# Richard-coder/uvio

Hardware: AMD Instinct MI355X
Metric: VIO frames/sec (track+propagate+update) at clones x feats (higher is better)
Workload: dtype f64

## Files before the change

include/uvio_hp.h:

```cpp
#ifndef UVIO_HP_H
#define UVIO_HP_H

#include <stddef.h>
#include <stdint.h>

#ifdef __cplusplus
extern "C" {
#endif

#define UVIO_HP_OK 0
#define UVIO_HP_E_ARG (-1)
#define UVIO_HP_E_STATE (-2)
#define UVIO_HP_E_DEVICE (-3)
#define UVIO_HP_E_NUMERIC (-4)
#define UVIO_HP_E_CONFIG (-5)
#define UVIO_HP_E_ORDER (-6)
#define UVIO_HP_E_CAPACITY (-7)
#define UVIO_HP_E_INTERNAL (-8)

#define UVIO_HP_MAX_CAMS 4
#define UVIO_HP_MAX_ANCHORS 16
#define UVIO_HP_AUX_MAX_DIM 8


// ... 208 lines not shown
int uvio_hp_aux_init_p(double *P, int N, int ld, int dim, const int *H_index, int n, const double *H_x, int ldhx,
                       const double *H_auxinv, const double *res_unused_or_null, const double *R, int ldr);
int uvio_hp_aux_walk_p(double *P, int N, int ld, int ntab, const int *ids, const int *dims, const double *sigma2,
                       double dt);
int uvio_hp_debug_position_update_p(double *P, int N, int ld, int imu_id, const double *q, const double *p, int aux_id,
                                    const double *s, int r, const double *C, const double *z, const double *R, int ldr,
                                    double chi2_thr, double *dx, double *chi2, int *applied);
int uvio_hp_chi2_95(int dof, double *thr);
int uvio_hp_msckf_compressed_update(double *P, int N, const int *H_index, int n, const double *H, int m,
                                    const double *res, double sigma2, double *dx_out);
int uvio_hp_compress(const double *A, int m, int n, double *R_out);
int uvio_hp_undistort(int model, const double cam[8], int n, const float *uv, float *uvn, uint8_t *ambiguous);
int uvio_hp_debug_grid_order(const uint8_t *resp, const int *off, int ncell, int kmax, int depth, int *arrangement,
                             int *top);
int uvio_hp_debug_clahe(const uint8_t *img, int w, int h, int stride, uint8_t *out);
typedef struct {
  uint64_t id;
  float u, v;
  int highlighted;
  int n_cams;
  int to_delete;
  int hist_off, hist_n;
} uvio_hp_viz_track_t;
int uvio_hp_debug_draw_tracks(int ncam, const uint8_t *const *imgs, const int *w, const int *h, const int *strides,
                              const uint8_t *const *masks, const int *counts, const uvio_hp_viz_track_t *tracks,
                              const float *uv, int n_uv, uint8_t *out, size_t cap, int *width, int *height,
                              double *stage_ms);
int uvio_hp_debug_loop_depth(const uint8_t *img, int w, int h, int stride, int n, const uint64_t *ids,
                             const double *uvd, uint16_t *depth, uint8_t *viz);
int uvio_hp_debug_track_image_times(uvio_hp_t *h, int on, double ms[5]);
// ... 7 lines not shown
```

uvio_amd/_native.py:

```python
import ctypes as C
import os

ROOT = os.path.dirname(os.path.dirname(os.path.abspath(__file__)))
LIB_PATH = os.environ.get("UVIO_HP_LIB", os.path.join(ROOT, "uvio_amd", "libuvio_hp.so"))

MAX_CAMS = 4
MAX_ANCHORS = 16
AUX_MAX_DIM = 8

OK = 0
E_ARG, E_STATE, E_DEVICE, E_NUMERIC, E_CONFIG, E_ORDER, E_CAPACITY, E_INTERNAL = -1, -2, -3, -4, -5, -6, -7, -8
ERRNAMES = {0: "OK", -1: "E_ARG", -2: "E_STATE", -3: "E_DEVICE", -4: "E_NUMERIC", -5: "E_CONFIG", -6: "E_ORDER",
            -7: "E_CAPACITY", -8: "E_INTERNAL"}


class Camera(C.Structure):
    _fields_ = [("model", C.c_int), ("width", C.c_int), ("height", C.c_int), ("intrinsics", C.c_double * 8),
                ("q_ItoC", C.c_double * 4), ("p_IinC", C.c_double * 3)]


class Anchor(C.Structure):
    _fields_ = [("id", C.c_uint64), ("fix", C.c_int), ("p_AinG", C.c_double * 3), ("const_bias", C.c_double),
                ("dist_bias", C.c_double), ("cov_diag", C.c_double * 5)]

# ... 115 lines not shown
    ("set_state", _I, [C.c_void_p, _P(_D), _P(_D), _I, _P(_D), _I, _I]),
    ("propagate_and_clone", _I, [C.c_void_p, _D]),
    ("msckf_update", _I, [C.c_void_p, _I, _P(C.c_uint64), _P(_I), _P(FeatMeas), _P(FeatResult)]),
    ("slam_update", _I, [C.c_void_p, _I, _P(C.c_uint64), _P(_I), _P(FeatMeas), _P(FeatResult)]),
    ("slam_delayed_init", _I, [C.c_void_p, _I, _P(C.c_uint64), _P(_I), _P(FeatMeas), _P(FeatResult)]),
    ("slam_change_anchors", _I, [C.c_void_p]),
    ("marginalize_slam", _I, [C.c_void_p]),
    ("marginalize_old_clone", _I, [C.c_void_p]),
    ("uwb_update_single", _I, [C.c_void_p, _D, C.c_uint64, _D, _P(_I)]),
    ("shard_unique_id", _I, [_P(C.c_uint8)]),
    ("shard_init_rccl", _I, [C.c_void_p, _I, _I, _P(C.c_uint8), _I]),
    ("shard_init_host", _I, [C.c_void_p, _I, _I, C.c_void_p, C.c_void_p, _I]),
    ("shard_partition", _I, [_P(_I), _I, _I, _P(_I)]),
    ("debug_grid_order", _I, [_P(C.c_uint8), _P(_I), _I, _I, _I, _P(_I), _P(_I)]),
    ("debug_clahe", _I, [_P(C.c_uint8), _I, _I, _I, _P(C.c_uint8)]),
    ("debug_grid_stats", _I, [C.c_void_p, _P(C.c_uint64), _P(C.c_uint64)]),
    ("get_marginal_cov", _I, [C.c_void_p, _I, _P(_I), _P(_I), _P(_D), _I]),
    ("get_good_features_msckf", _I, [C.c_void_p, _P(_D), _I, _P(_I)]),
    ("odometry_enable", _I, [C.c_void_p, _I]),
    ("fast_state_propagate", _I, [C.c_void_p, _D, _P(_D), _P(_D), _P(_I)]),
    ("get_track_image", _I, [C.c_void_p, _P(C.c_uint8), C.c_size_t, _P(_I), _P(_I), _P(_I)]),
    ("get_track_image_device", _I, [C.c_void_p, C.c_void_p, C.c_size_t, _P(_I), _P(_I), _P(_I)]),
    ("get_track_history", _I, [C.c_void_p, _I, C.c_uint64, _P(C.c_float), _I, _P(_I), _P(_I), _P(_I)]),
    ("get_loop_depth", _I, [C.c_void_p, _P(C.c_uint16), _P(C.c_uint8), C.c_size_t, _P(_I), _P(_I), _P(_D)]),
    ("debug_draw_tracks", _I, [_I, _P(_P(C.c_uint8)), _P(_I), _P(_I), _P(_I), _P(_P(C.c_uint8)), _P(_I),
                               _P(VizTrack), _P(C.c_float), _I, _P(C.c_uint8), C.c_size_t, _P(_I), _P(_I), _P(_D)]),
    ("debug_loop_depth", _I, [_P(C.c_uint8), _I, _I, _I, _I, _P(C.c_uint64), _P(_D), _P(C.c_uint16), _P(C.c_uint8)]),
    ("debug_track_image_times", _I, [C.c_void_p, _I, _P(_D)]),
    ("propagate", _I, [C.c_void_p, _D]),
    ("measurement_update", _I, [C.c_void_p, _I, _P(_I), _P(_I), _P(_D), _I, _I, _P(_D), _P(_D), _I, _D, _P(_D), _P(_I),
# ... 70 lines not shown
```

uvio_amd/csrc/capi.cpp:

```cpp
#include <cstring>
#include <string>

#include "engine.h"

using namespace uvhp;

struct uvio_hp {
  Engine *e = nullptr;
  std::string err;
  std::string fatal;
};

static std::string internal_error(const uvio_hp *h, const std::exception &ex) {
  std::string m = std::string("internal error: ") + ex.what();
  if (h && h->e && h->e->stage()[0]) m += std::string(" (in ") + h->e->stage() + ")";
  return m;
}

#define HP_GUARD(h, body)                                    \
  try {                                                      \
    if ((h) && (h)->e) HP_HIP(hipSetDevice((h)->e->device())); \
    body                                                     \
  } catch (const HpError &ex) {                              \
    if (h) (h)->err = ex.what();                             \
// ... 574 lines not shown
  } catch (...) {
    return UVIO_HP_E_DEVICE;
  }
}

int uvio_hp_debug_clahe(const uint8_t *img, int w, int h, int stride, uint8_t *out) {
  try {
    return Engine::clahe_standalone(img, w, h, stride, out);
  } catch (const HpError &ex) {
    return ex.code;
  } catch (...) {
    return UVIO_HP_E_DEVICE;
  }
}

int uvio_hp_debug_grid_stats(uvio_hp_t *h, uint64_t *cells, uint64_t *introsort_cells) {
  if (!h) return UVIO_HP_E_ARG;
  unsigned long long c = 0;
  unsigned long long i = 0;
  HP_GUARD(h, if (h->e->tracker()) h->e->tracker()->grid_stats(&c, &i);)
  if (cells) *cells = c;
  if (introsort_cells) *introsort_cells = i;
  return 0;
}

}
```

uvio_amd/csrc/engine.h:

```cpp
#pragma once
#include <chrono>
#include <atomic>
#include <functional>
#include <map>
#include <memory>
#include <mutex>
#include <stdexcept>
#include <unordered_map>
#include <algorithm>
#include <cstdlib>
#include <vector>

#include "hp_common.h"
#include "fast_prop.h"
#include "hprof.h"
#include "imu_math.h"
#include "kernels.h"
#include "pool.h"
#include "tracker.h"

namespace uvhp {

enum VKind { V_IMU = 0, V_VEC = 1, V_QUAT = 2, V_POSE = 3, V_LANDMARK = 4, V_ANCHOR = 5, V_AUX = 6 };

// ... 389 lines not shown
  void kernel_stats(bool flush, uvio_hp_kstat_t *out, int cap, int *n);

  void shard_init_rccl(int rank, int world, const uint8_t id[128], int min_features);
  void shard_init_host(int rank, int world, uvio_hp_allreduce_fn fn, void *user, int min_features);

  static int ekf_update_R_standalone(double *P, int N, const int *H_index, int n, const double *H, int r,
                                     const double *res, const double *R, int ldr, double chi2_thr, double *dx_out,
                                     double *chi2, int *applied);
  static int ekf_update_standalone(double *P, int N, const int *H_index, int n, const double *H, int r, const double *res,
                                   double sigma2, double *dx_out, bool compress = false);
  static int compress_standalone(const double *A, int m, int n, double *R_out);
  static int undistort_standalone(int model, const double cam[8], int n, const float *uv, float *uvn, uint8_t *amb);
  static int grid_order_standalone(const uint8_t *resp, const int *off, int ncell, int kmax, int depth,
                                   int *arrangement, int *top);
  static int clahe_standalone(const uint8_t *img, int w, int h, int stride, uint8_t *out);
  static int aux_append_standalone(double *P, int N, int ld, int dim, const double *prior, int ldp);
  static int aux_init_standalone(double *P, int N, int ld, int dim, const int *H_index, int n, const double *H_x,
                                 int ldhx, const double *H_auxinv, const double *R, int ldr);
  static int aux_walk_standalone(double *P, int N, int ld, int ntab, const int *ids, const int *dims,
                                 const double *sigma2, double dt);
  static int position_update_standalone(double *P, int N, int ld, int imu_id, const double *q, const double *p,
                                        int aux_id, const double *s, int r, const double *C, const double *z,
                                        const double *R, int ldr, double chi2_thr, double *dx, double *chi2,
                                        int *applied);

 private:
  uvio_hp_options_t o_;
  int device_;
  DeviceBufs d_;
  double timestamp_ = -1;
// ... 318 lines not shown
```

uvio_amd/csrc/engine_state.cpp:

```cpp
#include <sys/stat.h>

#include <algorithm>
#include <cstdio>
#include <cstring>

#include "engine.h"

namespace uvhp {

void Var::update(const double *dx) {
  if (kind == V_IMU || kind == V_POSE || kind == V_QUAT) {
    quat_boxplus(val, dx);
    for (int i = 3; i < size; i++) val[i + 1] += dx[i];
  } else {
    for (int i = 0; i < size; i++) val[i] += dx[i];
  }
}

void Var::xyz(bool getfej, double *o) const { landmark_get_xyz(rep, val, fej, uvn0, getfej, o); }
void Var::set_xyz(const double *p, bool isfej) {
  landmark_set_from_xyz(rep, p, isfej ? fej : val, isfej ? uvn0_fej : uvn0);
}

void MeasList::keep_if_valid(const std::vector<double> &valid) {
// ... 838 lines not shown
  job.p[0].w[0] = w;
  job.p[0].h[0] = h;
  job.p[0].img[0] = d_img;
  job.p[0].der[0] = d_der;
  job.src[0] = d_src;
  job.stride[0] = w;
  job.clahe[0] = d_lut;
  HP_HIP(hipMemcpy2DAsync(d_src, w, img, stride, w, h, hipMemcpyHostToDevice, s));
  launch_pyramids(s, job);
  HP_HIP(hipGetLastError());
  HP_HIP(hipMemcpyAsync(out, d_img, n, hipMemcpyDeviceToHost, s));
  HP_HIP(hipStreamSynchronize(s));
  return 0;
}

bool aux_upper_ok(const double *A, int ld, int d, bool pos_diag) {
  for (int i = 0; i < d; i++) {
    for (int j = i; j < d; j++)
      if (!std::isfinite(A[(size_t)i * ld + j])) return false;
    if (pos_diag && !(A[(size_t)i * ld + i] > 0.0)) return false;
  }
  return true;
}

bool aux_inverse(const double *A0, int lda, int d, double *inv) {
  double A[UVIO_HP_AUX_MAX_DIM * UVIO_HP_AUX_MAX_DIM], amax = 0.0;
  for (int i = 0; i < d; i++)
    for (int j = 0; j < d; j++) {
      const double v = A0[(size_t)i * lda + j];
      if (!std::isfinite(v)) return false;
// ... 183 lines not shown
```

uvio_amd/csrc/kernels.h:

```cpp
#pragma once
#include <hip/hip_runtime.h>

#include <cstdint>
#include <cstdlib>
#include <cstring>
#include <string>

#include "dev_mem.h"
#include "hp_math.h"
#include "kprof.h"

namespace uvhp {

constexpr int kMaxMeasPerFeat = 64;
constexpr int kMaxVarsPerFeat = 48;
constexpr int kMaxCams = 4;

struct DClone {
  double R[9], p[3];
  double Rf[9], pf[3];
  int pid;
  int canon;
  int pad[2];
};

// ... 297 lines not shown
void launch_subpix_multi(hipStream_t s, const SubpixJob &job, float *pts, const float *mask, int win, int max_iters,
                         double eps2);
void launch_subpix(hipStream_t s, const uint8_t *img, int w, int h, float *pts, int n, const float *mask, int win,
                   int max_iters, double eps2);
struct LkSlots {
  DPyr prev[kMaxCams], next[kMaxCams];
  const float *p0[kMaxCams];
  float *p1[kMaxCams];
  uint8_t *st[kMaxCams];
  int n[kMaxCams];
  unsigned long long *bytes = nullptr;
  CamParams c0[kMaxCams], c1[kMaxCams];
  float *p0n[kMaxCams] = {}, *p1n[kMaxCams] = {};
  uint8_t *p1amb[kMaxCams] = {};
  int undistort = 0;
};
void launch_undistort_points(hipStream_t s, const CamParams &cam, int n, const float *uv, float *uvn, uint8_t *amb);
void launch_lk(hipStream_t s, const LkSlots &job, int nslot, int win, int max_level, int max_iters, float eps,
               bool init_from_p0);
struct RansacSlots {
  CamParams c0[kMaxCams], c1[kMaxCams];
  const float *p0[kMaxCams], *p1[kMaxCams];
  float *p0n[kMaxCams], *p1n[kMaxCams];
  const int *sub[kMaxCams];
  double *F[kMaxCams];
  int *nm[kMaxCams], *good[kMaxCams];
  uint8_t *mask[kMaxCams];
  float t[kMaxCams];
  int n[kMaxCams];
};
void launch_ransac(hipStream_t s, const RansacSlots &job, int nslot, int max_iters, double conf,
                   bool undistorted = false);

enum VizKind { VIZ_DISC1 = 0, VIZ_DISC2 = 1, VIZ_SEG = 2, VIZ_RECT = 3, VIZ_FILL = 4 };
// ... 24 lines not shown
```

uvio_amd/csrc/kernels_track.hip:

```cpp
#include <cstdlib>
#include <stdexcept>
#include <utility>

#include "kernels.h"

namespace uvhp {

__device__ __forceinline__ int xcd_contiguous(int w, int nwg) {
  const int q = nwg / 8, r = nwg % 8, x = w % 8;
  return (x < r ? x * (q + 1) : r * (q + 1) + (x - r) * q) + w / 8;
}

__device__ __forceinline__ int reflect101(int p, int n) {
  if (n == 1) return 0;
  while (p < 0 || p >= n) p = (p < 0) ? -p : 2 * n - 2 - p;
  return p;
}

constexpr int kPM = 4;
template <int PW, int PH>
struct PairTile {
  static constexpr int WW = PW + 2 * kPM, WH = PH + 2 * kPM, QW = PW / 2, QH = PH / 2;
  static constexpr int SW = 2 * WW + 4, SH = 2 * WH + 4, PPT = PW * PH / 256;
};
// ... 996 lines not shown
#pragma unroll
  for (int k = 0; k < N; k++) d[k] += dpp_i32<0xB1>(d[k]);
#pragma unroll
  for (int k = 0; k < N; k++) d[k] += dpp_i32<0x4E>(d[k]);
#pragma unroll
  for (int k = 0; k < N; k++) d[k] += dpp_i32<0x141>(d[k]);
#pragma unroll
  for (int k = 0; k < N; k++) d[k] += dpp_i32<0x140>(d[k]);
#pragma unroll
  for (int k = 0; k < N; k++)
    out[k] = ((long long)__builtin_amdgcn_readlane(d[k], 0) + (long long)__builtin_amdgcn_readlane(d[k], 16)) +
             ((long long)__builtin_amdgcn_readlane(d[k], 32) + (long long)__builtin_amdgcn_readlane(d[k], 48));
}
constexpr int kLkMargin = 4, kLkMaxWin = 16, kLkMaxTile = kLkMaxWin + 1 + 2 * kLkMargin;
static_assert(kLkMaxWin * kLkMaxWin <= 4 * 64, "wave_sum_rows_i32 bound: at most 4 window pixels per lane");
#ifdef UVHP_LK_PROF
struct LkProf {
  unsigned long long setup, stage, iter, total;
  int n_iter, n_stage, n_level, pad;
};
__device__ LkProf g_lk_prof[4096];
#define LKP_T(v) const unsigned long long v = clock64()
#else
#define LKP_T(v)
#endif
__device__ __forceinline__ float2 lk_point(const DPyr &prev, const DPyr &next, const float *__restrict__ p0,
                                         float *__restrict__ p1, uint8_t *__restrict__ status, int pi, int win,
                                         int max_level, int max_iters, float crit_eps, int init_from_p0,
                                         unsigned long long *bytes) {
  const int lane = threadIdx.x;
  const int maxL = min(max_level, min(prev.levels, next.levels) - 1);
  const float halfw = (win - 1) * 0.5f;
  const float FLT_SCALE = 1.f / (1 << 20);
  const float WSCALE = (float)(1 << 14);
  const int area = win * win;
  constexpr int kPer = 4;
  int Iw[kPer], dIx[kPer], dIy[kPer];
  __shared__ uint8_t Jt[kLkMaxTile * kLkMaxTile];
  const int S = win + 1 + 2 * kLkMargin;
  int wx[kPer], wy[kPer], jo[kPer];
#pragma unroll
  for (int q = 0; q < kPer; q++) {
    const int e = min(lane + 64 * q, area - 1);
    wy[q] = e / win;
    wx[q] = e - wy[q] * win;
    jo[q] = wy[q] * S + wx[q];
  }
  constexpr int kStageN = (kLkMaxTile * kLkMaxTile + 63) / 64;
  int sx[kStageN], sy[kStageN];
#pragma unroll
  for (int k = 0; k < kStageN; k++) {
    const int e = min(lane + 64 * k, S * S - 1);
    sy[k] = e / S;
    sx[k] = e - sy[k] * S;
  }
  float qx = init_from_p0 ? p0[2 * pi] : p1[2 * pi], qy = init_from_p0 ? p0[2 * pi + 1] : p1[2 * pi + 1];
  uint8_t st = 1;
  int nlev = 0, nit = 0;
#ifdef UVHP_LK_PROF
  unsigned long long c_setup = 0, c_stage = 0, c_iter = 0;
  int n_stage = 0;
  LKP_T(c_begin);
#endif
  const float p0x = p0[2 * pi], p0y = p0[2 * pi + 1];
  int gi[kPer][4], gd[kPer][4], gm[kPer];
  auto gather = [&](int l) {
    const uint8_t *I = prev.img[l];
    const int *d32 = reinterpret_cast<const int *>(prev.der[l]);
    const int Iw_ = prev.w[l], Ih_ = prev.h[l];
    const float sc = (float)(1. / (1 << l));
    float prx = p0x * sc, pry = p0y * sc;
    prx -= halfw;
    pry -= halfw;
    const int ipx = min(max((int)floorf(prx), -win), Iw_ - 1), ipy = min(max((int)floorf(pry), -win), Ih_ - 1);
    if (ipx >= 0 && ipx + win < Iw_ && ipy >= 0 && ipy + win < Ih_) {
#pragma unroll
// ... 19 lines not shown
      gi[q][0] = I[ry0 + rx0];
      gi[q][1] = I[ry0 + rx1];
      gi[q][2] = I[ry1 + rx0];
      gi[q][3] = I[ry1 + rx1];
      const int cx0 = min(max(X, 0), Iw_ - 1), cx1 = min(max(X + 1, 0), Iw_ - 1);
      const size_t cy0 = (size_t)min(max(Y, 0), Ih_ - 1) * Iw_, cy1 = (size_t)min(max(Y + 1, 0), Ih_ - 1) * Iw_;
      gd[q][0] = d32[cy0 + cx0];
      gd[q][1] = d32[cy0 + cx1];
      gd[q][2] = d32[cy1 + cx0];
      gd[q][3] = d32[cy1 + cx1];
      const bool vx0 = X >= 0 && X < Iw_, vx1 = X + 1 >= 0 && X + 1 < Iw_;
      const bool vy0 = Y >= 0 && Y < Ih_, vy1 = Y + 1 >= 0 && Y + 1 < Ih_;
      gm[q] = (vx0 && vy0) | (vx1 && vy0) << 1 | (vx0 && vy1) << 2 | (vx1 && vy1) << 3;
    }
  };
  if (maxL >= 0) gather(maxL);
  for (int level = maxL; level >= 0; level--) {
    const uint8_t *J = next.img[level];
    const int Iw_ = prev.w[level], Ih_ = prev.h[level], Jw_ = next.w[level], Jh_ = next.h[level];
    const float sc = (float)(1. / (1 << level));
    float prx = p0x * sc, pry = p0y * sc;
    if (level == maxL) {
      qx = qx * sc;
      qy = qy * sc;
    } else {
      qx = qx * 2.f;
      qy = qy * 2.f;
    }
    prx -= halfw;
    pry -= halfw;
    LKP_T(c_l0);
    const int ipx = (int)floorf(prx), ipy = (int)floorf(pry);
    if (ipx < -win || ipx >= Iw_ || ipy < -win || ipy >= Ih_) {
      if (level == 0) st = 0;
      if (level > 0) gather(level - 1);
      continue;
    }
    float a = prx - ipx, b = pry - ipy;
    int iw00 = (int)rintf((1.f - a) * (1.f - b) * WSCALE);
    int iw01 = (int)rintf(a * (1.f - b) * WSCALE);
    int iw10 = (int)rintf((1.f - a) * b * WSCALE);
    int iw11 = (1 << 14) - iw00 - iw01 - iw10;
    int sA11 = 0, sA12 = 0, sA22 = 0;
#pragma unroll
    for (int q = 0; q < kPer; q++) {
      const int ival = descale(dot4_i24(gi[q][0], gi[q][1], gi[q][2], gi[q][3], iw00, iw01, iw10, iw11), 14 - 5);
#pragma unroll
      for (int k = 0; k < 4; k++)
        if (!(gm[q] >> k & 1)) gd[q][k] = 0;
      auto lo = [](int v) { return (int)(int16_t)(v & 0xffff); };
      auto hi = [](int v) { return v >> 16; };
      const int ixv = descale(dot4_i24(lo(gd[q][0]), lo(gd[q][1]), lo(gd[q][2]), lo(gd[q][3]), iw00, iw01, iw10, iw11), 14);
      const int iyv = descale(dot4_i24(hi(gd[q][0]), hi(gd[q][1]), hi(gd[q][2]), hi(gd[q][3]), iw00, iw01, iw10, iw11), 14);
      const bool in = lane + 64 * q < area;
      Iw[q] = in ? (int16_t)ival : 0;
      dIx[q] = in ? (int16_t)ixv : 0;
      dIy[q] = in ? (int16_t)iyv : 0;
      sA11 += dIx[q] * dIx[q];
      sA12 += dIx[q] * dIy[q];
      sA22 += dIy[q] * dIy[q];
    }
    if (level > 0) gather(level - 1);
    long long s3[3];
    wave_sum_rows_i32<3>({sA11, sA12, sA22}, s3);
    const float A11 = (float)s3[0] * FLT_SCALE, A12 = (float)s3[1] * FLT_SCALE, A22 = (float)s3[2] * FLT_SCALE;
    float D = A11 * A22 - A12 * A12;
    const float minEig = (A22 + A11 - sqrtf((A11 - A22) * (A11 - A22) + 4.f * A12 * A12)) / (float)(2 * win * win);
    if (minEig < 1e-4f || D < 1.19209290e-07f) {
      if (level == 0) st = 0;
      continue;
    }
    D = 1.f / D;
    nlev++;
#ifdef UVHP_LK_PROF
    c_setup += clock64() - c_l0;
#endif
    float nx = qx - halfw, ny = qy - halfw;
    float pdx = 0.f, pdy = 0.f;
    int ox = -(1 << 28), oy = -(1 << 28);
    for (int j = 0; j < max_iters; j++) {
      LKP_T(c_i0);
      const int inx = (int)floorf(nx), iny = (int)floorf(ny);
      if (inx < -win || inx >= Jw_ || iny < -win || iny >= Jh_) {
        if (level == 0) st = 0;
        break;
      }
      if (inx - ox < 0 || inx - ox > 2 * kLkMargin || iny - oy < 0 || iny - oy > 2 * kLkMargin) {
        __syncthreads();
        ox = inx - kLkMargin;
        oy = iny - kLkMargin;
        uint8_t v[kStageN];
        if (ox >= 0 && ox + S <= Jw_ && oy >= 0 && oy + S <= Jh_) {
#pragma unroll
          for (int k = 0; k < kStageN; k++) v[k] = J[(size_t)(oy + sy[k]) * Jw_ + ox + sx[k]];
        } else {
#pragma unroll
          for (int k = 0; k < kStageN; k++) v[k] = J[(size_t)reflect101(oy + sy[k], Jh_) * Jw_ + reflect101(ox + sx[k], Jw_)];
        }
#pragma unroll
        for (int k = 0; k < kStageN; k++)
          if (lane + 64 * k < S * S) Jt[lane + 64 * k] = v[k];
        __syncthreads();
#ifdef UVHP_LK_PROF
        c_stage += clock64() - c_i0;
        n_stage++;
#endif
      }
      a = nx - inx;
      b = ny - iny;
      iw00 = (int)rintf((1.f - a) * (1.f - b) * WSCALE);
      iw01 = (int)rintf(a * (1.f - b) * WSCALE);
      iw10 = (int)rintf((1.f - a) * b * WSCALE);
      iw11 = (1 << 14) - iw00 - iw01 - iw10;
      int ib1 = 0, ib2 = 0;
      nit++;
      const uint8_t *t0 = Jt + (iny - oy) * S + (inx - ox);
      int tp[kPer][4];
#pragma unroll
      for (int q = 0; q < kPer; q++) {
        const uint8_t *t = t0 + jo[q];
        tp[q][0] = t[0];
// ... 19 lines not shown
#ifdef UVHP_LK_PROF
      c_iter += clock64() - c_i0;
#endif
      const float e2 = dx * dx + dy * dy;
      bool conv = e2 < crit_eps * 0.9999f;
      if (!conv && !(e2 > crit_eps * 1.0001f)) conv = (double)dx * dx + (double)dy * dy <= (double)crit_eps;
      if (conv) break;
      if (j > 0 && fabsf(dx + pdx) < 0.01f && fabsf(dy + pdy) < 0.01f) {
        qx -= dx * 0.5f;
        qy -= dy * 0.5f;
        break;
      }
      pdx = dx;
      pdy = dy;
    }
  }
  if (lane == 0) {
    p1[2 * pi] = qx;
    p1[2 * pi + 1] = qy;
    status[pi] = st;
    if (bytes) atomicAdd(bytes, (unsigned long long)(256 * (5 * nlev + nit)));
#ifdef UVHP_LK_PROF
    if (pi < 4096) g_lk_prof[pi] = LkProf{c_setup, c_stage, c_iter - c_stage, clock64() - c_begin, nit, n_stage, nlev, 0};
#endif
  }
  return make_float2(qx, qy);
}

__global__ void __launch_bounds__(64) k_lk(LkSlots job, int win, int max_level, int max_iters, float crit_eps,
                                           int init_from_p0) {
  const int idx = xcd_contiguous(blockIdx.x + blockIdx.y * gridDim.x, gridDim.x * gridDim.y);
  const int slot = idx / gridDim.x, p = idx - slot * gridDim.x;
  if (p >= job.n[slot]) return;
  const float2 q = lk_point(job.prev[slot], job.next[slot], job.p0[slot], job.p1[slot], job.st[slot], p, win,
                            max_level, max_iters, crit_eps, init_from_p0, job.bytes);
  if (job.undistort && threadIdx.x < 2) {
    const int w = threadIdx.x;
    const float px = w ? q.x : job.p0[slot][2 * p], py = w ? q.y : job.p0[slot][2 * p + 1];
    float x, y;
    const bool amb = cam_undistort_f(w ? job.c1[slot] : job.c0[slot], px, py, x, y);
    float *out = w ? job.p1n[slot] : job.p0n[slot];
    out[2 * p] = x;
    out[2 * p + 1] = y;
    if (w && job.p1amb[slot]) job.p1amb[slot][p] = amb ? 1 : 0;
  }
}

__global__ void __launch_bounds__(256) k_undistort_points(CamParams cam, int n, const float *__restrict__ uv,
                                                          float *__restrict__ uvn, uint8_t *__restrict__ amb) {
  const int p = blockIdx.x * blockDim.x + threadIdx.x;
  if (p >= n) return;
  float x, y;
// ... 318 lines not shown
      throw std::runtime_error("cornerSubPix window outside the kernel's 1..5 instantiations");
  }
}

void launch_subpix(hipStream_t s, const uint8_t *img, int w, int h, float *pts, int n, const float *mask, int win,
                   int max_iters, double eps2) {
  SubpixJob job{};
  job.img[0] = img;
  job.w[0] = w;
  job.h[0] = h;
  job.end[0] = n;
  job.ncam = 1;
  launch_subpix_multi(s, job, pts, mask, win, max_iters, eps2);
}

void launch_lk(hipStream_t s, const LkSlots &job, int nslot, int win, int max_level, int max_iters, float eps,
               bool init_from_p0) {
  int nmax = 0;
  for (int k = 0; k < nslot; k++) nmax = max(nmax, job.n[k]);
  if (nmax <= 0) return;
  if (win > kLkMaxWin) throw std::runtime_error("LK window larger than the kernel supports");
  hipLaunchKernelGGL(k_lk, dim3(nmax, nslot), dim3(64), 0, s, job, win, max_level, max_iters, eps * eps,
                     init_from_p0 ? 1 : 0);
}

void launch_ransac(hipStream_t s, const RansacSlots &job, int nslot, int max_iters, double conf, bool undistorted) {
  int nmax = 0;
  for (int k = 0; k < nslot; k++) nmax = max(nmax, job.n[k]);
  if (nmax <= 0) return;
  if (!undistorted) hipLaunchKernelGGL(k_undistort, dim3((nmax + 127) / 128, 2 * nslot), dim3(128), 0, s, job);
  hipLaunchKernelGGL(k_ransac_hyp, dim3((max_iters + 3) / 4, nslot), dim3(256), 0, s, job, max_iters);
  hipLaunchKernelGGL(k_ransac_select, dim3(1, nslot), dim3(256), 0, s, job, max_iters, conf);
}

}
```

uvio_amd/manager.py:

```python
import ctypes as C

import numpy as np

from . import _native as N


def load_options(yaml_path=None, **overrides):
    lib = N.load()
    opts = N.Options()
    N.check(lib.uvio_hp_options_default(C.byref(opts)), what="options_default")
    if yaml_path is not None:
        N.check(lib.uvio_hp_options_load(yaml_path.encode(), C.byref(opts)), what="options_load(%s)" % yaml_path)
    apply_overrides(opts, overrides)
    return opts


def _mask_ptrs(masks, ncam):
    mk = [None if m is None else np.ascontiguousarray(m, dtype=np.uint8) for m in masks]
    ptrs = [C.POINTER(C.c_uint8)() if m is None else m.ctypes.data_as(C.POINTER(C.c_uint8)) for m in mk]
    return mk, (C.POINTER(C.c_uint8) * ncam)(*ptrs)


def apply_overrides(opts, overrides):
    for k, v in overrides.items():
# ... 808 lines not shown
def clahe(img):
    lib = N.load()
    img = np.asarray(img)
    if img.ndim != 2 or img.dtype != np.uint8:
        raise ValueError("clahe: a 2-D uint8 image")
    if img.strides[1] != 1 or img.strides[0] < img.shape[1]:
        img = np.ascontiguousarray(img)
    h, w = img.shape
    out = np.zeros((h, w), dtype=np.uint8)
    bp = C.POINTER(C.c_uint8)
    rc = lib.uvio_hp_debug_clahe(img.ctypes.data_as(bp), w, h, img.strides[0], out.ctypes.data_as(bp))
    N.check(rc, what="uvio_hp_debug_clahe")
    return out


def undistort(cam, uv, return_ambiguous=False):
    lib = N.load()
    uv = np.ascontiguousarray(uv, dtype=np.float32).reshape(-1, 2)
    out = np.zeros_like(uv)
    amb = np.zeros(uv.shape[0], dtype=np.uint8)
    intr = np.array(cam.intrinsics[:], dtype=np.float64)
    fp = C.POINTER(C.c_float)
    rc = lib.uvio_hp_undistort(int(cam.model), _dp(intr), uv.shape[0], uv.ctypes.data_as(fp), out.ctypes.data_as(fp),
                               amb.ctypes.data_as(C.POINTER(C.c_uint8)))
    N.check(rc, what="uvio_hp_undistort")
    return (out, amb) if return_ambiguous else out
```

Measured before the change: 1118.

## Pipeline LK pyramid levels across multiple waves per feature workgroup

The LK tracking kernel becomes a template over W waves per workgroup. Each wave owns a subset of pyramid levels, gathers its level's template and Hessian ahead of time, and receives the coarser level's flow estimate through an LDS handoff with workgroup-scope flags. A launcher picks W from occupancy queries, so more waves are used only when the point count fits in resident workgroups. The aim is to overlap per-level setup and gathers across waves and raise latency hiding when few features are tracked, at the cost of spin-waits, extra LDS and a more complex kernel. It also adds debug entry points for standalone LK and for inspecting the schedule.

```diff
diff --git a/include/uvio_hp.h b/include/uvio_hp.h
--- a/include/uvio_hp.h
+++ b/include/uvio_hp.h
@@ -246,6 +246,10 @@
 int uvio_hp_debug_grid_order(const uint8_t *resp, const int *off, int ncell, int kmax, int depth, int *arrangement,
                              int *top);
 int uvio_hp_debug_clahe(const uint8_t *img, int w, int h, int stride, uint8_t *out);
+int uvio_hp_debug_lk(const uint8_t *prev, const uint8_t *next, int w, int h, int n, const float *p0, float *p1,
+                     uint8_t *status, int win, int max_level, int max_iters, float eps, int waves, int *counters,
+                     int *waves_used);
+int uvio_hp_debug_lk_schedule(int levels, int waves, int *owner, int *turn, int *waits_for);
 typedef struct {
   uint64_t id;
   float u, v;
diff --git a/uvio_amd/_native.py b/uvio_amd/_native.py
--- a/uvio_amd/_native.py
+++ b/uvio_amd/_native.py
@@ -153,6 +153,9 @@
     ("shard_partition", _I, [_P(_I), _I, _I, _P(_I)]),
     ("debug_grid_order", _I, [_P(C.c_uint8), _P(_I), _I, _I, _I, _P(_I), _P(_I)]),
     ("debug_clahe", _I, [_P(C.c_uint8), _I, _I, _I, _P(C.c_uint8)]),
+    ("debug_lk", _I, [_P(C.c_uint8), _P(C.c_uint8), _I, _I, _I, _P(C.c_float), _P(C.c_float), _P(C.c_uint8), _I, _I, _I,
+                      C.c_float, _I, _P(_I), _P(_I)]),
+    ("debug_lk_schedule", _I, [_I, _I, _P(_I), _P(_I), _P(_I)]),
     ("debug_grid_stats", _I, [C.c_void_p, _P(C.c_uint64), _P(C.c_uint64)]),
     ("get_marginal_cov", _I, [C.c_void_p, _I, _P(_I), _P(_I), _P(_D), _I]),
     ("get_good_features_msckf", _I, [C.c_void_p, _P(_D), _I, _P(_I)]),
diff --git a/uvio_amd/csrc/capi.cpp b/uvio_amd/csrc/capi.cpp
--- a/uvio_amd/csrc/capi.cpp
+++ b/uvio_amd/csrc/capi.cpp
@@ -612,6 +612,35 @@
   }
 }
 
+int uvio_hp_debug_lk(const uint8_t *prev, const uint8_t *next, int w, int h, int n, const float *p0, float *p1,
+                     uint8_t *status, int win, int max_level, int max_iters, float eps, int waves, int *counters,
+                     int *waves_used) {
+  try {
+    return Engine::lk_standalone(prev, next, w, h, n, p0, p1, status, win, max_level, max_iters, eps, waves, counters,
+                                 waves_used);
+  } catch (const HpError &ex) {
+    return ex.code;
+  } catch (...) {
+    return UVIO_HP_E_DEVICE;
+  }
+}
+
+int uvio_hp_debug_lk_schedule(int levels, int waves, int *owner, int *turn, int *waits_for) {
+  if (levels < 1 || levels > uvhp::kMaxPyrLevels || waves < 1 || waves > uvhp::kLkMaxWaves || !owner || !turn || !waits_for)
+    return UVIO_HP_E_ARG;
+  const int maxL = levels - 1;
+  for (int l = 0; l < levels; l++) owner[l] = turn[l] = waits_for[l] = -1;
+  for (int w = 0; w < waves; w++)
+    for (int k = 0; uvhp::lk_wave_level(maxL, w, waves, k) >= 0; k++) {
+      const int l = uvhp::lk_wave_level(maxL, w, waves, k);
+      if (owner[l] >= 0 || uvhp::lk_owner(maxL, l, waves) != w) return UVIO_HP_E_DEVICE;
+      owner[l] = w;
+      turn[l] = k;
+      waits_for[l] = uvhp::lk_waits_for(maxL, l);
+    }
+  return 0;
+}
+
 int uvio_hp_debug_grid_stats(uvio_hp_t *h, uint64_t *cells, uint64_t *introsort_cells) {
   if (!h) return UVIO_HP_E_ARG;
   unsigned long long c = 0;
diff --git a/uvio_amd/csrc/engine.h b/uvio_amd/csrc/engine.h
--- a/uvio_amd/csrc/engine.h
+++ b/uvio_amd/csrc/engine.h
@@ -427,6 +427,9 @@
   static int grid_order_standalone(const uint8_t *resp, const int *off, int ncell, int kmax, int depth,
                                    int *arrangement, int *top);
   static int clahe_standalone(const uint8_t *img, int w, int h, int stride, uint8_t *out);
+  static int lk_standalone(const uint8_t *prev, const uint8_t *next, int w, int h, int n, const float *p0, float *p1,
+                           uint8_t *status, int win, int max_level, int max_iters, float eps, int waves, int *counters,
+                           int *waves_used);
   static int aux_append_standalone(double *P, int N, int ld, int dim, const double *prior, int ldp);
   static int aux_init_standalone(double *P, int N, int ld, int dim, const int *H_index, int n, const double *H_x,
                                  int ldhx, const double *H_auxinv, const double *R, int ldr);
diff --git a/uvio_amd/csrc/engine_state.cpp b/uvio_amd/csrc/engine_state.cpp
--- a/uvio_amd/csrc/engine_state.cpp
+++ b/uvio_amd/csrc/engine_state.cpp
@@ -876,6 +876,80 @@
   return 0;
 }
 
+int Engine::lk_standalone(const uint8_t *prev, const uint8_t *next, int w, int h, int n, const float *p0, float *p1,
+                          uint8_t *status, int win, int max_level, int max_iters, float eps, int waves, int *counters,
+                          int *waves_used) {
+  if (!prev || !next || w < 1 || h < 1 || n < 0 || (n > 0 && (!p0 || !p1 || !status))) return UVIO_HP_E_ARG;
+  if (win < 1 || win > 16 || max_level < 0 || max_level >= kMaxPyrLevels || max_iters < 0 || !(eps >= 0.f) || waves < 0 ||
+      waves > kLkMaxWaves)
+    return UVIO_HP_E_ARG;
+  if (w > 16384 || h > 16384 || n > (1 << 20)) return UVIO_HP_E_CAPACITY;
+  int ndev = 0;
+  if (hipGetDeviceCount(&ndev) != hipSuccess || ndev < 1) return UVIO_HP_E_DEVICE;
+  Stream s = Stream::create();
+  DPyr shape{};
+  size_t bytes = 0;
+  std::vector<size_t> img_off, der_off;
+  for (int level = 0, lw = w, lh = h; level <= max_level; level++) {
+    shape.w[level] = lw;
+    shape.h[level] = lh;
+    shape.levels = level + 1;
+    img_off.push_back(bytes);
+    bytes += ((size_t)lw * lh + 255) & ~(size_t)255;
+    der_off.push_back(bytes);
+    bytes += ((size_t)lw * lh * 4 + 255) & ~(size_t)255;
+    lw = (lw + 1) / 2;
+    lh = (lh + 1) / 2;
+    if (lw <= win || lh <= win) break;
+  }
+  const size_t npix = (size_t)w * h, np = (size_t)std::max(n, 1);
+  DevBuf<char> mem[2] = {DevBuf<char>(bytes), DevBuf<char>(bytes)};
+  DevBuf<uint8_t> d_src(2 * npix), d_st(np);
+  DevBuf<unsigned> d_hist(512);
+  DevBuf<float> d_p0(2 * np), d_p1(2 * np);
+  DevBuf<int> d_cnt(2 * np);
+  PyrJob job{};
+  job.ncam = 2;
+  job.method = 0;
+  for (int k = 0; k < 2; k++) {
+    job.p[k] = shape;
+    for (int l = 0; l < shape.levels; l++) {
+      job.p[k].img[l] = (const uint8_t *)((char *)mem[k] + img_off[l]);
+      job.p[k].der[l] = (const int16_t *)((char *)mem[k] + der_off[l]);
+    }
+    job.src[k] = (uint8_t *)d_src + k * npix;
+    job.stride[k] = w;
+    job.hist[k] = (unsigned *)d_hist + 256 * k;
+  }
+  HP_HIP(hipMemcpyAsync(d_src, prev, npix, hipMemcpyHostToDevice, s));
+  HP_HIP(hipMemcpyAsync((uint8_t *)d_src + npix, next, npix, hipMemcpyHostToDevice, s));
+  HP_HIP(hipMemsetAsync(d_hist, 0, 512 * sizeof(unsigned), s));
+  launch_pyramids(s, job);
+  HP_HIP(hipGetLastError());
+  const int levels = std::min(max_level, shape.levels - 1) + 1;
+  if (waves_used) *waves_used = lk_waves_for(levels, n, waves);
+  if (n > 0) {
+    HP_HIP(hipMemcpyAsync(d_p0, p0, 2 * sizeof(float) * (size_t)n, hipMemcpyHostToDevice, s));
+    HP_HIP(hipMemcpyAsync(d_p1, p1, 2 * sizeof(float) * (size_t)n, hipMemcpyHostToDevice, s));
+    HP_HIP(hipMemsetAsync(d_cnt, 0, 2 * sizeof(int) * (size_t)n, s));
+    LkSlots lk{};
+    lk.prev[0] = job.p[0];
+    lk.next[0] = job.p[1];
+    lk.p0[0] = d_p0;
+    lk.p1[0] = d_p1;
+    lk.st[0] = d_st;
+    lk.n[0] = n;
+    lk.dbg[0] = d_cnt;
+    launch_lk(s, lk, 1, win, max_level, max_iters, eps, false, waves);
+    HP_HIP(hipGetLastError());
+    HP_HIP(hipMemcpyAsync(p1, d_p1, 2 * sizeof(float) * (size_t)n, hipMemcpyDeviceToHost, s));
+    HP_HIP(hipMemcpyAsync(status, d_st, (size_t)n, hipMemcpyDeviceToHost, s));
+    if (counters) HP_HIP(hipMemcpyAsync(counters, d_cnt, 2 * sizeof(int) * (size_t)n, hipMemcpyDeviceToHost, s));
+  }
+  HP_HIP(hipStreamSynchronize(s));
+  return 0;
+}
+
 bool aux_upper_ok(const double *A, int ld, int d, bool pos_diag) {
   for (int i = 0; i < d; i++) {
     for (int j = i; j < d; j++)
diff --git a/uvio_amd/csrc/kernels.h b/uvio_amd/csrc/kernels.h
--- a/uvio_amd/csrc/kernels.h
+++ b/uvio_amd/csrc/kernels.h
@@ -9,6 +9,7 @@
 #include "dev_mem.h"
 #include "hp_math.h"
 #include "kprof.h"
+#include "lk_schedule.h"
 
 namespace uvhp {
 
@@ -336,10 +337,12 @@
   float *p0n[kMaxCams] = {}, *p1n[kMaxCams] = {};
   uint8_t *p1amb[kMaxCams] = {};
   int undistort = 0;
+  int *dbg[kMaxCams] = {};
 };
 void launch_undistort_points(hipStream_t s, const CamParams &cam, int n, const float *uv, float *uvn, uint8_t *amb);
 void launch_lk(hipStream_t s, const LkSlots &job, int nslot, int win, int max_level, int max_iters, float eps,
-               bool init_from_p0);
+               bool init_from_p0, int force_waves = 0);
+int lk_waves_for(int levels, int points, int force_waves = 0);
 struct RansacSlots {
   CamParams c0[kMaxCams], c1[kMaxCams];
   const float *p0[kMaxCams], *p1[kMaxCams];
diff --git a/uvio_amd/csrc/kernels_track.hip b/uvio_amd/csrc/kernels_track.hip
--- a/uvio_amd/csrc/kernels_track.hip
+++ b/uvio_amd/csrc/kernels_track.hip
@@ -1034,29 +1034,53 @@
 }
 constexpr int kLkMargin = 4, kLkMaxWin = 16, kLkMaxTile = kLkMaxWin + 1 + 2 * kLkMargin;
 static_assert(kLkMaxWin * kLkMaxWin <= 4 * 64, "wave_sum_rows_i32 bound: at most 4 window pixels per lane");
+struct LkHand {
+  float qx, qy;
+  int nlev, nit, nrest, nspec, bad;
+  int flag;
+};
+constexpr unsigned kLkSpinMax = 1u << 20;
 #ifdef UVHP_LK_PROF
 struct LkProf {
-  unsigned long long setup, stage, iter, total;
-  int n_iter, n_stage, n_level, pad;
+  unsigned long long setup, wait, stage, iter, total;
+  int n_iter, n_stage, n_level, n_spec;
 };
-__device__ LkProf g_lk_prof[4096];
+__device__ LkProf g_lk_prof[4096 * kLkMaxWaves];
 #define LKP_T(v) const unsigned long long v = clock64()
 #else
 #define LKP_T(v)
 #endif
+template <int W>
+__device__ __forceinline__ void lk_wave_sync() {
+  if constexpr (W == 1) {
+    __syncthreads();
+  } else {
+    wave_lds_sync();
+  }
+}
+template <int W>
 __device__ __forceinline__ float2 lk_point(const DPyr &prev, const DPyr &next, const float *__restrict__ p0,
                                          float *__restrict__ p1, uint8_t *__restrict__ status, int pi, int win,
                                          int max_level, int max_iters, float crit_eps, int init_from_p0,
-                                         unsigned long long *bytes) {
-  const int lane = threadIdx.x;
+                                         unsigned long long *bytes, int *dbg, bool &fin) {
+  const int lane = W == 1 ? threadIdx.x : (threadIdx.x & 63);
+  const int wv = W == 1 ? 0 : uni(threadIdx.x >> 6);
   const int maxL = min(max_level, min(prev.levels, next.levels) - 1);
+  fin = false;
+  __shared__ LkHand hand[W > 1 ? kMaxPyrLevels : 1];
+  if constexpr (W > 1) {
+    if (threadIdx.x < kMaxPyrLevels) hand[threadIdx.x].flag = 0;
+    __syncthreads();
+    if (maxL - wv < 0 && !(maxL < 0 && wv == 0)) return make_float2(0.f, 0.f);
+  }
   const float halfw = (win - 1) * 0.5f;
   const float FLT_SCALE = 1.f / (1 << 20);
   const float WSCALE = (float)(1 << 14);
   const int area = win * win;
   constexpr int kPer = 4;
   int Iw[kPer], dIx[kPer], dIy[kPer];
-  __shared__ uint8_t Jt[kLkMaxTile * kLkMaxTile];
+  __shared__ uint8_t Jt_all[W][kLkMaxTile * kLkMaxTile];
+  uint8_t *const Jt = Jt_all[wv];
   const int S = win + 1 + 2 * kLkMargin;
   int wx[kPer], wy[kPer], jo[kPer];
 #pragma unroll
@@ -1075,11 +1099,13 @@
     sx[k] = e - sy[k] * S;
   }
   float qx = init_from_p0 ? p0[2 * pi] : p1[2 * pi], qy = init_from_p0 ? p0[2 * pi + 1] : p1[2 * pi + 1];
+  const float q0x = qx, q0y = qy;
   uint8_t st = 1;
   int nlev = 0, nit = 0;
+  int nrest = 0, nspec = 0, bad = 0;
 #ifdef UVHP_LK_PROF
-  unsigned long long c_setup = 0, c_stage = 0, c_iter = 0;
-  int n_stage = 0;
+  unsigned long long c_setup = 0, c_wait = 0, c_stage = 0, c_iter = 0;
+  int n_stage = 0, n_own = 0;
   LKP_T(c_begin);
 #endif
   const float p0x = p0[2 * pi], p0y = p0[2 * pi + 1];
@@ -1129,97 +1155,154 @@
       gm[q] = (vx0 && vy0) | (vx1 && vy0) << 1 | (vx0 && vy1) << 2 | (vx1 && vy1) << 3;
     }
   };
-  if (maxL >= 0) gather(maxL);
-  for (int level = maxL; level >= 0; level--) {
+  constexpr int kNoTile = -(1 << 28);
+  int ox = kNoTile, oy = kNoTile;
+  auto tile_miss = [&](int inx, int iny) {
+    return inx - ox < 0 || inx - ox > 2 * kLkMargin || iny - oy < 0 || iny - oy > 2 * kLkMargin;
+  };
+  auto stage = [&](const uint8_t *J, int Jw_, int Jh_, int inx, int iny) {
+    lk_wave_sync<W>();
+    ox = inx - kLkMargin;
+    oy = iny - kLkMargin;
+    uint8_t v[kStageN];
+    if (ox >= 0 && ox + S <= Jw_ && oy >= 0 && oy + S <= Jh_) {
+#pragma unroll
+      for (int k = 0; k < kStageN; k++) v[k] = J[(size_t)(oy + sy[k]) * Jw_ + ox + sx[k]];
+    } else {
+#pragma unroll
+      for (int k = 0; k < kStageN; k++) v[k] = J[(size_t)reflect101(oy + sy[k], Jh_) * Jw_ + reflect101(ox + sx[k], Jw_)];
+    }
+#pragma unroll
+    for (int k = 0; k < kStageN; k++)
+      if (lane + 64 * k < S * S) Jt[lane + 64 * k] = v[k];
+    lk_wave_sync<W>();
+  };
+  auto stage_guess = [&](const uint8_t *J, int Jw_, int Jh_, float gx, float gy) {
+    const int inx = uni((int)floorf(gx - halfw)), iny = uni((int)floorf(gy - halfw));
+    if (inx < -win || inx >= Jw_ || iny < -win || iny >= Jh_) return;
+    if (tile_miss(inx, iny)) stage(J, Jw_, Jh_, inx, iny);
+  };
+  if (maxL - wv >= 0) gather(maxL - wv);
+  for (int level = maxL - wv; level >= 0; level -= W) {
     const uint8_t *J = next.img[level];
     const int Iw_ = prev.w[level], Ih_ = prev.h[level], Jw_ = next.w[level], Jh_ = next.h[level];
     const float sc = (float)(1. / (1 << level));
     float prx = p0x * sc, pry = p0y * sc;
-    if (level == maxL) {
-      qx = qx * sc;
-      qy = qy * sc;
-    } else {
-      qx = qx * 2.f;
-      qy = qy * 2.f;
-    }
     prx -= halfw;
     pry -= halfw;
     LKP_T(c_l0);
     const int ipx = (int)floorf(prx), ipy = (int)floorf(pry);
-    if (ipx < -win || ipx >= Iw_ || ipy < -win || ipy >= Ih_) {
-      if (level == 0) st = 0;
-      if (level > 0) gather(level - 1);
-      continue;
-    }
+    bool run = !(ipx < -win || ipx >= Iw_ || ipy < -win || ipy >= Ih_);
     float a = prx - ipx, b = pry - ipy;
     int iw00 = (int)rintf((1.f - a) * (1.f - b) * WSCALE);
     int iw01 = (int)rintf(a * (1.f - b) * WSCALE);
     int iw10 = (int)rintf((1.f - a) * b * WSCALE);
     int iw11 = (1 << 14) - iw00 - iw01 - iw10;
     int sA11 = 0, sA12 = 0, sA22 = 0;
-#pragma unroll
-    for (int q = 0; q < kPer; q++) {
-      const int ival = descale(dot4_i24(gi[q][0], gi[q][1], gi[q][2], gi[q][3], iw00, iw01, iw10, iw11), 14 - 5);
-#pragma unroll
-      for (int k = 0; k < 4; k++)
-        if (!(gm[q] >> k & 1)) gd[q][k] = 0;
-      auto lo = [](int v) { return (int)(int16_t)(v & 0xffff); };
-      auto hi = [](int v) { return v >> 16; };
-      const int ixv = descale(dot4_i24(lo(gd[q][0]), lo(gd[q][1]), lo(gd[q][2]), lo(gd[q][3]), iw00, iw01, iw10, iw11), 14);
-      const int iyv = descale(dot4_i24(hi(gd[q][0]), hi(gd[q][1]), hi(gd[q][2]), hi(gd[q][3]), iw00, iw01, iw10, iw11), 14);
-      const bool in = lane + 64 * q < area;
-      Iw[q] = in ? (int16_t)ival : 0;
-      dIx[q] = in ? (int16_t)ixv : 0;
-      dIy[q] = in ? (int16_t)iyv : 0;
-      sA11 += dIx[q] * dIx[q];
-      sA12 += dIx[q] * dIy[q];
-      sA22 += dIy[q] * dIy[q];
-    }
-    if (level > 0) gather(level - 1);
-    long long s3[3];
-    wave_sum_rows_i32<3>({sA11, sA12, sA22}, s3);
-    const float A11 = (float)s3[0] * FLT_SCALE, A12 = (float)s3[1] * FLT_SCALE, A22 = (float)s3[2] * FLT_SCALE;
-    float D = A11 * A22 - A12 * A12;
-    const float minEig = (A22 + A11 - sqrtf((A11 - A22) * (A11 - A22) + 4.f * A12 * A12)) / (float)(2 * win * win);
-    if (minEig < 1e-4f || D < 1.19209290e-07f) {
-      if (level == 0) st = 0;
-      continue;
-    }
-    D = 1.f / D;
-    nlev++;
+    if (run) {
+#pragma unroll
+      for (int q = 0; q < kPer; q++) {
+        const int ival = descale(dot4_i24(gi[q][0], gi[q][1], gi[q][2], gi[q][3], iw00, iw01, iw10, iw11), 14 - 5);
+#pragma unroll
+        for (int k = 0; k < 4; k++)
+          if (!(gm[q] >> k & 1)) gd[q][k] = 0;
+        auto lo = [](int v) { return (int)(int16_t)(v & 0xffff); };
+        auto hi = [](int v) { return v >> 16; };
+        const int ixv = descale(dot4_i24(lo(gd[q][0]), lo(gd[q][1]), lo(gd[q][2]), lo(gd[q][3]), iw00, iw01, iw10, iw11), 14);
+        const int iyv = descale(dot4_i24(hi(gd[q][0]), hi(gd[q][1]), hi(gd[q][2]), hi(gd[q][3]), iw00, iw01, iw10, iw11), 14);
+        const bool in = lane + 64 * q < area;
+        Iw[q] = in ? (int16_t)ival : 0;
+        dIx[q] = in ? (int16_t)ixv : 0;
+        dIy[q] = in ? (int16_t)iyv : 0;
+        sA11 += dIx[q] * dIx[q];
+        sA12 += dIx[q] * dIy[q];
+        sA22 += dIy[q] * dIy[q];
+      }
+    }
+    if (level - W >= 0) gather(level - W);
+    float A11 = 0.f, A12 = 0.f, A22 = 0.f, D = 0.f;
+    if (run) {
+      long long s3[3];
+      wave_sum_rows_i32<3>({sA11, sA12, sA22}, s3);
+      A11 = (float)s3[0] * FLT_SCALE, A12 = (float)s3[1] * FLT_SCALE, A22 = (float)s3[2] * FLT_SCALE;
+      D = A11 * A22 - A12 * A12;
+      const float minEig = (A22 + A11 - sqrtf((A11 - A22) * (A11 - A22) + 4.f * A12 * A12)) / (float)(2 * win * win);
+      if (minEig < 1e-4f || D < 1.19209290e-07f)
+        run = false;
+      else
+        D = 1.f / D;
+    }
 #ifdef UVHP_LK_PROF
     c_setup += clock64() - c_l0;
+    n_own++;
 #endif
+    ox = oy = kNoTile;
+    if (level == maxL) {
+      qx = q0x * sc;
+      qy = q0y * sc;
+    } else if constexpr (W == 1) {
+      qx = qx * 2.f;
+      qy = qy * 2.f;
+    } else {
+      LKP_T(c_w0);
+      if (run) stage_guess(J, Jw_, Jh_, q0x * sc, q0y * sc);
+      int seen = maxL + 1;
+      unsigned spins = 0;
+      bool gave_up = false;
+      while (!__hip_atomic_load(&hand[level + 1].flag, __ATOMIC_RELAXED, __HIP_MEMORY_SCOPE_WORKGROUP)) {
+        for (int k = level + 2; run && k < seen; k++)
+          if (__hip_atomic_load(&hand[k].flag, __ATOMIC_RELAXED, __HIP_MEMORY_SCOPE_WORKGROUP)) {
+            __builtin_amdgcn_fence(__ATOMIC_ACQUIRE, "workgroup");
+            const float m = (float)(1 << (k - level));
+            stage_guess(J, Jw_, Jh_, hand[k].qx * m, hand[k].qy * m);
+            seen = k;
+            break;
+          }
+        __builtin_amdgcn_s_sleep(1);
+        if (++spins > kLkSpinMax) {
+          gave_up = true;
+          break;
+        }
+      }
+      __builtin_amdgcn_fence(__ATOMIC_ACQUIRE, "workgroup");
+      if (!gave_up) {
+        const LkHand &h = hand[level + 1];
+        qx = __int_as_float(uni(__float_as_int(h.qx))) * 2.f;
+        qy = __int_as_float(uni(__float_as_int(h.qy))) * 2.f;
+        nlev = uni(h.nlev);
+        nit = uni(h.nit);
+        nrest = uni(h.nrest);
+        nspec = uni(h.nspec);
+        bad = uni(h.bad);
+      } else {
+        bad = 1;
+        qx = q0x * sc;
+        qy = q0y * sc;
+      }
+#ifdef UVHP_LK_PROF
+      c_wait += clock64() - c_w0;
+#endif
+    }
+    if (!run && level == 0) st = 0;
+    if (run) nlev++;
     float nx = qx - halfw, ny = qy - halfw;
     float pdx = 0.f, pdy = 0.f;
-    int ox = -(1 << 28), oy = -(1 << 28);
-    for (int j = 0; j < max_iters; j++) {
+    for (int j = 0; run && j < max_iters; j++) {
       LKP_T(c_i0);
       const int inx = (int)floorf(nx), iny = (int)floorf(ny);
       if (inx < -win || inx >= Jw_ || iny < -win || iny >= Jh_) {
         if (level == 0) st = 0;
         break;
       }
-      if (inx - ox < 0 || inx - ox > 2 * kLkMargin || iny - oy < 0 || iny - oy > 2 * kLkMargin) {
-        __syncthreads();
-        ox = inx - kLkMargin;
-        oy = iny - kLkMargin;
-        uint8_t v[kStageN];
-        if (ox >= 0 && ox + S <= Jw_ && oy >= 0 && oy + S <= Jh_) {
-#pragma unroll
-          for (int k = 0; k < kStageN; k++) v[k] = J[(size_t)(oy + sy[k]) * Jw_ + ox + sx[k]];
-        } else {
-#pragma unroll
-          for (int k = 0; k < kStageN; k++) v[k] = J[(size_t)reflect101(oy + sy[k], Jh_) * Jw_ + reflect101(ox + sx[k], Jw_)];
-        }
-#pragma unroll
-        for (int k = 0; k < kStageN; k++)
-          if (lane + 64 * k < S * S) Jt[lane + 64 * k] = v[k];
-        __syncthreads();
+      if (tile_miss(inx, iny)) {
+        if (ox != kNoTile) nrest++;
+        stage(J, Jw_, Jh_, inx, iny);
 #ifdef UVHP_LK_PROF
         c_stage += clock64() - c_i0;
         n_stage++;
 #endif
+      } else if (W > 1 && j == 0) {
+        nspec++;
       }
       a = nx - inx;
       b = ny - iny;
@@ -1269,28 +1352,46 @@
       pdx = dx;
       pdy = dy;
     }
-  }
-  if (lane == 0) {
+    if (level == 0) {
+      fin = true;
+    } else if constexpr (W > 1) {
+      if (lane == 0) {
+        LkHand &h = hand[level];
+        h.qx = qx, h.qy = qy;
+        h.nlev = nlev, h.nit = nit, h.nrest = nrest, h.nspec = nspec, h.bad = bad;
+      }
+      __builtin_amdgcn_fence(__ATOMIC_RELEASE, "workgroup");
+      if (lane == 0) __hip_atomic_store(&hand[level].flag, 1, __ATOMIC_RELAXED, __HIP_MEMORY_SCOPE_WORKGROUP);
+    }
+  }
+  if (maxL < 0) fin = true;
+  if (fin && lane == 0) {
     p1[2 * pi] = qx;
     p1[2 * pi + 1] = qy;
-    status[pi] = st;
+    status[pi] = bad ? 255 : st;
     if (bytes) atomicAdd(bytes, (unsigned long long)(256 * (5 * nlev + nit)));
+    if (dbg) dbg[2 * pi] = nrest, dbg[2 * pi + 1] = nspec;
+  }
 #ifdef UVHP_LK_PROF
-    if (pi < 4096) g_lk_prof[pi] = LkProf{c_setup, c_stage, c_iter - c_stage, clock64() - c_begin, nit, n_stage, nlev, 0};
+  if (lane == 0 && pi < 4096)
+    g_lk_prof[pi * kLkMaxWaves + wv] =
+        LkProf{c_setup, c_wait, c_stage, c_iter - c_stage, clock64() - c_begin, fin ? nit : 0, n_stage, n_own, fin ? nspec : 0};
 #endif
-  }
   return make_float2(qx, qy);
 }
 
-__global__ void __launch_bounds__(64) k_lk(LkSlots job, int win, int max_level, int max_iters, float crit_eps,
-                                           int init_from_p0) {
+template <int W>
+__global__ void __launch_bounds__(64 * W) k_lk(LkSlots job, int win, int max_level, int max_iters, float crit_eps,
+                                               int init_from_p0) {
   const int idx = xcd_contiguous(blockIdx.x + blockIdx.y * gridDim.x, gridDim.x * gridDim.y);
   const int slot = idx / gridDim.x, p = idx - slot * gridDim.x;
   if (p >= job.n[slot]) return;
-  const float2 q = lk_point(job.prev[slot], job.next[slot], job.p0[slot], job.p1[slot], job.st[slot], p, win,
-                            max_level, max_iters, crit_eps, init_from_p0, job.bytes);
-  if (job.undistort && threadIdx.x < 2) {
-    const int w = threadIdx.x;
+  bool fin;
+  const float2 q = lk_point<W>(job.prev[slot], job.next[slot], job.p0[slot], job.p1[slot], job.st[slot], p, win,
+                               max_level, max_iters, crit_eps, init_from_p0, job.bytes, job.dbg[slot], fin);
+  const int lane = W == 1 ? threadIdx.x : (threadIdx.x & 63);
+  if (job.undistort && fin && lane < 2) {
+    const int w = lane;
     const float px = w ? q.x : job.p0[slot][2 * p], py = w ? q.y : job.p0[slot][2 * p + 1];
     float x, y;
     const bool amb = cam_undistort_f(w ? job.c1[slot] : job.c0[slot], px, py, x, y);
@@ -1639,14 +1740,57 @@
   launch_subpix_multi(s, job, pts, mask, win, max_iters, eps2);
 }
 
+template <int W>
+static void lk_query_resident(int cus, int (&r)[kLkMaxWaves + 1]) {
+  int nb = 0;
+  if (hipOccupancyMaxActiveBlocksPerMultiprocessor(&nb, (const void *)k_lk<W>, 64 * W, 0) != hipSuccess) nb = 0;
+  r[W] = nb * cus;
+  if constexpr (W > 1) lk_query_resident<W - 1>(cus, r);
+}
+static const int (&lk_resident_workgroups())[kLkMaxWaves + 1] {
+  static const struct Res {
+    int r[kLkMaxWaves + 1] = {};
+    Res() {
+      int dev = 0, cus = 0;
+      if (hipGetDevice(&dev) != hipSuccess ||
+          hipDeviceGetAttribute(&cus, hipDeviceAttributeMultiprocessorCount, dev) != hipSuccess)
+        cus = 0;
+      lk_query_resident<kLkMaxWaves>(cus, r);
+    }
+  } res;
+  return res.r;
+}
+static int lk_waves_control() {
+  static const int v = [] {
+    const char *e = std::getenv("UVIO_HP_LK_WAVES");
+    const int w = e ? std::atoi(e) : 0;
+    return w > 0 ? min(w, kLkMaxWaves) : 0;
+  }();
+  return v;
+}
+int lk_waves_for(int levels, int points, int force_waves) {
+  return lk_pick_waves(levels, points, lk_resident_workgroups(), force_waves > 0 ? force_waves : lk_waves_control());
+}
+template <int W>
+static void lk_launch_w(int w, hipStream_t s, dim3 grid, const LkSlots &job, int win, int max_level, int max_iters,
+                        float crit_eps, int init_from_p0) {
+  if (w == W)
+    hipLaunchKernelGGL(k_lk<W>, grid, dim3(64 * W), 0, s, job, win, max_level, max_iters, crit_eps, init_from_p0);
+  else if constexpr (W > 1)
+    lk_launch_w<W - 1>(w, s, grid, job, win, max_level, max_iters, crit_eps, init_from_p0);
+}
+
 void launch_lk(hipStream_t s, const LkSlots &job, int nslot, int win, int max_level, int max_iters, float eps,
-               bool init_from_p0) {
+               bool init_from_p0, int force_waves) {
   int nmax = 0;
   for (int k = 0; k < nslot; k++) nmax = max(nmax, job.n[k]);
   if (nmax <= 0) return;
   if (win > kLkMaxWin) throw std::runtime_error("LK window larger than the kernel supports");
-  hipLaunchKernelGGL(k_lk, dim3(nmax, nslot), dim3(64), 0, s, job, win, max_level, max_iters, eps * eps,
-                     init_from_p0 ? 1 : 0);
+  int levels = 0;
+  for (int k = 0; k < nslot; k++)
+    levels = max(levels, min(max_level, min(job.prev[k].levels, job.next[k].levels) - 1) + 1);
+  const int W = lk_waves_for(levels, nmax * nslot, force_waves);
+  lk_launch_w<kLkMaxWaves>(W, s, dim3(nmax, nslot), job, win, max_level, max_iters, eps * eps, init_from_p0 ? 1 : 0);
 }
 
 void launch_ransac(hipStream_t s, const RansacSlots &job, int nslot, int max_iters, double conf, bool undistorted) {
diff --git a/uvio_amd/csrc/lk_schedule.h b/uvio_amd/csrc/lk_schedule.h
--- /dev/null
+++ b/uvio_amd/csrc/lk_schedule.h
@@ -0,0 +1,21 @@
+#pragma once
+
+namespace uvhp {
+
+constexpr int kLkMaxWaves = 6;
+
+constexpr int lk_owner(int maxL, int l, int W) { return (maxL - l) % W; }
+constexpr int lk_wave_level(int maxL, int w, int W, int k) { return maxL - w - k * W; }
+constexpr int lk_waits_for(int maxL, int l) { return l < maxL ? l + 1 : -1; }
+
+constexpr int kLkAutoMaxWaves = 4;
+
+inline int lk_pick_waves(int levels, int points, const int (&resident)[kLkMaxWaves + 1], int forced) {
+  if (forced > 0) return forced < kLkMaxWaves ? forced : kLkMaxWaves;
+  int W = 1;
+  for (int w = 2; w <= kLkAutoMaxWaves && w <= levels; w++)
+    if (points <= resident[w]) W = w;
+  return W;
+}
+
+}
diff --git a/uvio_amd/manager.py b/uvio_amd/manager.py
--- a/uvio_amd/manager.py
+++ b/uvio_amd/manager.py
@@ -846,6 +846,36 @@
     return out
 
 
+def lk(prev, nxt, p0, p1=None, win=15, max_level=5, max_iters=30, eps=0.01, waves=0):
+    lib = N.load()
+    prev = np.ascontiguousarray(prev, dtype=np.uint8)
+    nxt = np.ascontiguousarray(nxt, dtype=np.uint8)
+    if prev.ndim != 2 or prev.shape != nxt.shape:
+        raise ValueError("lk: two 2-D uint8 images of one size")
+    h, w = prev.shape
+    a = np.array(p0, dtype=np.float32, order="C").reshape(-1, 2)
+    b = np.array(a if p1 is None else p1, dtype=np.float32, order="C").reshape(-1, 2)
+    n = a.shape[0]
+    st = np.zeros(max(n, 1), dtype=np.uint8)
+    cnt = np.zeros((max(n, 1), 2), dtype=np.int32)
+    used = C.c_int(0)
+    bp, fp, ip = C.POINTER(C.c_uint8), C.POINTER(C.c_float), C.POINTER(C.c_int)
+    rc = lib.uvio_hp_debug_lk(prev.ctypes.data_as(bp), nxt.ctypes.data_as(bp), w, h, n, a.ctypes.data_as(fp),
+                              b.ctypes.data_as(fp), st.ctypes.data_as(bp), win, max_level, max_iters, eps, waves,
+                              cnt.ctypes.data_as(ip), C.byref(used))
+    N.check(rc, what="uvio_hp_debug_lk")
+    return b, st[:n], cnt[:n], used.value
+
+
+def lk_schedule(levels, waves):
+    lib = N.load()
+    o, t, wf = (np.zeros(levels, dtype=np.int32) for _ in range(3))
+    ip = C.POINTER(C.c_int)
+    rc = lib.uvio_hp_debug_lk_schedule(levels, waves, o.ctypes.data_as(ip), t.ctypes.data_as(ip), wf.ctypes.data_as(ip))
+    N.check(rc, what="uvio_hp_debug_lk_schedule")
+    return o, t, wf
+
+
 def undistort(cam, uv, return_ambiguous=False):
     lib = N.load()
     uv = np.ascontiguousarray(uv, dtype=np.float32).reshape(-1, 2)
```

Result: no change. 1129, median of 3 (+1.0%).
